# zju3dv/Mirror-NeRF

Measured on AMD Instinct MI355X. Metric: rendered rays/sec (primary+reflected), higher is better.
Workload: dtype f32 carried as hi/lo f16 pairs (f16 MFMA, f32 accumulate; max |diff| to the fp32 chain 3e-6)

## Files before the change

include/mnrf.h:

```cpp
#ifndef MNRF_H
#define MNRF_H

#include <stdint.h>

#ifdef __cplusplus
extern "C" {
#endif

#define MNRF_HOST

#define MNRF_OK 0
#define MNRF_ERR_ARG (-1)
#define MNRF_ERR_LAUNCH (-2)
#define MNRF_ERR_UNSUPPORTED (-3)

#define MNRF_N_PARAMS 32

#define MNRF_SIGMA_ONLY 1u
#define MNRF_GRAD_NORMAL 2u
#define MNRF_SPLIT_F16 4u

#define MNRF_TCNN_GRAD_F16 16u
#define MNRF_TCNN_GRAD_FIXED 512u
#define MNRF_TCNN_F16 256u
// ... 161 lines not shown
                     float bound, int64_t B, const float* xyz, int64_t xyz_stride, const float* rays, const float* z_vals,
                     int spr, float* planes, void* stream);

int mnrf_tcnn_encode_flags(const float* table, MNRF_HOST const int64_t* offsets17_host, double log2_per_level_scale, int base_resolution,
                           float bound, int64_t B, const float* xyz, int64_t xyz_stride, const float* rays, const float* z_vals,
                           int spr, float* planes, unsigned flags, void* stream);
int mnrf_tcnn_table_half(const float* table, int64_t entries, void* table_half, void* stream);

int mnrf_bench_gather(const void* table, int64_t table_bytes, int bytes_per_gather, int64_t n_threads, int iters, float* out,
                      void* stream);

#define MNRF_FUSED_WHITE_BACK 1u
#define MNRF_FUSED_RGB_DEPTH 2u
#define MNRF_FUSED_BLENDED_LEVEL 8u
int mnrf_fused_samples_per_ray(void);
int mnrf_field_composite_fused(float* packed, int64_t n_rays, const float* rays, const float* z_vals,
                               const float* dir_emb, int64_t dir_stride, int flags,
                               float* weights, float* opacity, float* rgb_map, float* depth, float* mirror_mask,
                               float* surf_normal, float* x_surface, void* stream);
int mnrf_field_composite_fused_pn(float* packed, int64_t n_rays, const float* rays, const float* z_vals,
                                  const float* dir_emb, int64_t dir_stride, int flags,
                                  float* weights, float* opacity, float* rgb_map, float* depth, float* mirror_mask,
                                  float* surf_normal, float* x_surface, float* pred_normal, void* stream);

int mnrf_split_convert_long(int on);
int mnrf_split2_probe(const float* x, int64_t n_pairs, int relu, int long_form, uint32_t* hi, uint32_t* lo, void* stream);

#define MNRF_TRAIN_PLANES 256u
#define MNRF_PLANES_Y_HALF 0x100000u
int64_t mnrf_train_planes_bytes(int64_t B);
int64_t mnrf_train_dy_planes_bytes(int64_t B);

int mnrf_field_backward_planes(float* packed, int64_t B, const float* xyz, int64_t xyz_stride,
                               const float* rays, const float* z_vals, int spr,
                               const float* g_sigma, const float* g_rgb, const float* g_pred_normal,
                               const float* g_is_mirror, const float* rgb, const float* pred_normal,
                               const float* is_mirror, const uint64_t* save_mask, const float* save_inv,
                               void* dy_planes, uint32_t* seedmax, float* d_xyz, float* d_dir, const float* keep_mirror,
                               unsigned flags ,
                               void* stream);

int64_t mnrf_dw_planes_workspace_floats(int n_eval, MNRF_HOST const int64_t* B);
int mnrf_dw_planes(int n_eval, const void* const* x_planes, const void* const* dy_planes, MNRF_HOST const int64_t* B,
                   const uint32_t* const* seedmax, float* workspace, float* const* d_params, int accumulate, void* stream);

int64_t mnrf_train_planes2_bytes(int64_t B);
// ... 310 lines not shown
```

mirror_nerf_amd/csrc/mnrf_render.hip:

```cpp
#include <hip/hip_runtime.h>
#include <stdint.h>
#include <stdio.h>
#include <string.h>

#include "../../include/mnrf.h"
#include "mnrf_error.h"
#include "mnrf_fill.h"
#include "mnrf_rays.h"

static thread_local char g_err[512] = "";

int mnrf_fail(int code, const char* msg) {
    snprintf(g_err, sizeof(g_err), "%s", msg);
    return code;
}

int mnrf_check_launch(const char* where) {
    hipError_t e = hipGetLastError();
    if (e != hipSuccess) {
        snprintf(g_err, sizeof(g_err), "%s: %s", where, hipGetErrorString(e));
        return MNRF_ERR_LAUNCH;
    }
    return MNRF_OK;
}

extern "C" const char* mnrf_last_error(void) { return g_err; }
extern "C" int mnrf_version(void) { return 1; }

namespace {

constexpr float EPS32 = 1.1920928955078125e-07f;

__device__ __forceinline__ long long live_rows(long long cap, const int* __restrict__ n_live) {
    if (!n_live) return cap;
    const long long v = *n_live;
    return v < 0 ? 0 : (v < cap ? v : cap);
}

__device__ __forceinline__ float wave_sum(float v) {
#pragma unroll
    for (int o = 32; o > 0; o >>= 1) v += __shfl_xor(v, o);
    return v;
}
#include "mnrf_composite.inc"

__global__ void embed_kernel(const float* __restrict__ x, long long n, int c, int n_freqs, float* __restrict__ out,
                             const int* __restrict__ n_live) {
    const long long i = (long long)blockIdx.x * blockDim.x + threadIdx.x;
    if (i >= live_rows(n, n_live) * c) return;
    const long long row = i / c;
    const int ch = (int)(i % c);
    const int ld = c * (2 * n_freqs + 1);
    const float v = x[i];
    float* o = out + row * ld;
    o[ch] = v;
    for (int f = 0; f < n_freqs; ++f) {
        float s, co;
        sincosf(ldexpf(v, f), &s, &co);
        o[c * (1 + 2 * f) + ch] = s;
        o[c * (2 + 2 * f) + ch] = co;
    }
}

__global__ void sample_coarse_kernel(const float* __restrict__ rays, long long n_rays, const float* __restrict__ z_steps,
                                     int ns, int use_disp, float perturb, const float* __restrict__ prand,
                                     float* __restrict__ z_out, const int* __restrict__ n_live) {
    const long long i = (long long)blockIdx.x * blockDim.x + threadIdx.x;
    if (i >= live_rows(n_rays, n_live) * ns) return;
    const long long r = i / ns;
    const int s = (int)(i % ns);
    const float near = rays[r * 8 + 6], far = rays[r * 8 + 7];
    auto zat = [&](int k) -> float {
        const float t = z_steps[k];
        if (!use_disp) return near * (1.f - t) + far * t;
        return 1.f / (1.f / near * (1.f - t) + 1.f / far * t);
    };
    float z = zat(s);
    if (perturb > 0.f) {
        const float lower = s == 0 ? z : 0.5f * (zat(s - 1) + z);
        const float upper = s == ns - 1 ? z : 0.5f * (z + zat(s + 1));
        z = lower + (upper - lower) * (perturb * prand[i]);
    }
    z_out[i] = z;
}

struct CompArgs {
    const float* rays; long long n_rays; int S;
    const float* sigma; const float* z; const float* noise; const float* rgb; const float* is_mirror;
    const float* pred_normal; const float* normal; int white_back;
    float* weights; float* opacity; float* rgb_map; float* depth; float* mirror_mask;
    float* surf_normal; float* surf_normal_grad; float* normal_dif; float* x_surface;
    const int* n_live;
};

struct CompGlobalSrc {
    const CompArgs& A;
    long long ray;
    __device__ __forceinline__ bool has_w() const { return false; }
    __device__ __forceinline__ float w(int) const { return 0.f; }
    __device__ __forceinline__ bool has_noise() const { return A.noise != nullptr; }
    __device__ __forceinline__ bool has_rgb() const { return A.rgb != nullptr; }
    __device__ __forceinline__ bool has_mirror() const { return A.is_mirror != nullptr; }
    __device__ __forceinline__ bool has_pn() const { return A.pred_normal != nullptr; }
    __device__ __forceinline__ bool has_gn() const { return A.normal != nullptr; }
    __device__ __forceinline__ float z(int s) const { return A.z[ray * A.S + s]; }
    __device__ __forceinline__ float sigma(int s) const { return A.sigma[ray * A.S + s]; }
// ... 242 lines not shown
    if (!live) ray = n_rays - 1;
    sample_fine_ray(z_coarse, weights, ray, live, S, u, u_per_ray, n_imp, z_fine);
}

__global__ __launch_bounds__(256) void composite_sample_kernel(CompArgs A, const float* __restrict__ u, int u_per_ray, int n_imp,
                                                               float* __restrict__ z_fine) {
    const int lane = threadIdx.x & 63;
    long long ray = (long long)blockIdx.x * 4 + (threadIdx.x >> 6);
    const long long n_rays = live_rows(A.n_rays, A.n_live);
    if ((long long)blockIdx.x * 4 >= n_rays) return;
    const bool live = ray < n_rays;
    if (live) {
        const CompGlobalSrc src{A, ray};
        const CompMaps out{A.weights + ray * A.S, A.opacity, A.rgb_map, A.depth, A.mirror_mask, A.surf_normal,
                           A.surf_normal_grad, A.normal_dif, A.x_surface, A.rays, A.white_back};
        composite_ray(src, A.S, lane, ray, out);
    }
    __threadfence_block();
    __syncthreads();
    if (!live) ray = n_rays - 1;
    sample_fine_ray(A.z, A.weights, ray, live, A.S, u, u_per_ray, n_imp, z_fine);
}

__global__ void threshold_kernel(float* __restrict__ m, long long n, int* __restrict__ any, const int* __restrict__ n_live) {
    const long long i = (long long)blockIdx.x * blockDim.x + threadIdx.x;
    bool nz = false;
    if (i < live_rows(n, n_live)) {
        float v = m[i];
        if (v > 0.5f) v = 1.f;
        else if (v < 0.5f) v = 0.f;
        m[i] = v;
        nz = v != 0.f;
    }
    if (__ballot(nz) != 0ull && (threadIdx.x & 63) == 0 && any) atomicOr(any, 1);
}

struct ReflArgs {
    const float* rays; const float* x_surface; const float* normal; const float* normal_noise; float noise_std;
    const float* mask; long long n; int compact; float near2;
    float* sec; int* index; int* count; float* reflect_dir;
    const int* n_live;
    int* slot;
};

__global__ __launch_bounds__(1024) void reflect_compact_kernel(ReflArgs A) {
    __shared__ int s_wave[16];
    __shared__ int s_base;
    const int tid = threadIdx.x, lane = tid & 63, wv = tid >> 6;
    if (tid == 0) s_base = 0;
    __syncthreads();
    A.n = live_rows(A.n, A.n_live);
    for (long long start = 0; start < A.n; start += 1024) {
        const long long i = start + tid;
// ... 24 lines not shown
        __syncthreads();
        int woff = 0, tot = 0;
        for (int k = 0; k < 16; ++k) { const int c = s_wave[k]; if (k < wv) woff += c; tot += c; }
        const int base = s_base;
        if (sel) {
            const long long p = base + woff + before;
            float* o = A.sec + p * 8;
            o[0] = A.x_surface[i * 3]; o[1] = A.x_surface[i * 3 + 1]; o[2] = A.x_surface[i * 3 + 2];
            o[3] = r[0]; o[4] = r[1]; o[5] = r[2];
            o[6] = A.near2;
            o[7] = A.rays[i * 8 + 7];
            A.index[p] = (int)i;
            if (A.slot) A.slot[i] = (int)p;
        } else if (in && A.slot) {
            A.slot[i] = -1;
        }
        __syncthreads();
        if (tid == 0) s_base = base + tot;
        __syncthreads();
    }
    if (tid == 0) *A.count = s_base;
}

__global__ __launch_bounds__(256) void reflect_all_kernel(ReflArgs A) {
    const long long i = (long long)blockIdx.x * blockDim.x + threadIdx.x;
    A.n = live_rows(A.n, A.n_live);
    if (i == 0) *A.count = (int)A.n;
    if (i >= A.n) return;
    float nv[3], wvv[3], r[3];
#pragma unroll
    for (int k = 0; k < 3; ++k) {
        nv[k] = A.normal[i * 3 + k];
        if (A.normal_noise) nv[k] = nv[k] + A.normal_noise[i * 3 + k] * A.noise_std;
        wvv[k] = -A.rays[i * 8 + 3 + k];
    }
    const float ninv = 1.f / sqrtf(fmaxf(nv[0] * nv[0] + nv[1] * nv[1] + nv[2] * nv[2], EPS32));
    const float winv = 1.f / sqrtf(fmaxf(wvv[0] * wvv[0] + wvv[1] * wvv[1] + wvv[2] * wvv[2], EPS32));
#pragma unroll
    for (int k = 0; k < 3; ++k) { nv[k] = nv[k] * ninv; wvv[k] = wvv[k] * winv; }
    const float c = wvv[0] * nv[0] + wvv[1] * nv[1] + wvv[2] * nv[2];
#pragma unroll
    for (int k = 0; k < 3; ++k) r[k] = 2.f * c * nv[k] - wvv[k];
    if (A.reflect_dir) { for (int k = 0; k < 3; ++k) A.reflect_dir[i * 3 + k] = r[k]; }
    float* o = A.sec + i * 8;
    o[0] = A.x_surface[i * 3]; o[1] = A.x_surface[i * 3 + 1]; o[2] = A.x_surface[i * 3 + 2];
    o[3] = r[0]; o[4] = r[1]; o[5] = r[2];
    o[6] = A.near2;
    o[7] = A.rays[i * 8 + 7];
    A.index[i] = (int)i;
    if (A.slot) A.slot[i] = (int)i;
}

__global__ void blend_all_kernel(const float* __restrict__ base, const float* __restrict__ sec, const float* __restrict__ mask,
                                 long long n, int c, int direct, float* __restrict__ out, float* __restrict__ refl,
                                 const int* __restrict__ n_live) {
    const long long i = (long long)blockIdx.x * blockDim.x + threadIdx.x;
    if (i >= live_rows(n, n_live) * c) return;
    const float m = mask[i / c];
    const float b = base[i];
    const float part = direct ? sec[i] : b;
    out[i] = m * part + (1.f - m) * b;
    if (refl) refl[i] = direct ? sec[i] : 0.f;
}

__global__ void blend_scatter_kernel(const float* __restrict__ base, const float* __restrict__ sec, const int* __restrict__ index,
                                     long long n_sec, const float* __restrict__ mask, int c, float* __restrict__ out,
                                     float* __restrict__ refl, const int* __restrict__ n_sec_live) {
    const long long j = (long long)blockIdx.x * blockDim.x + threadIdx.x;
    if (j >= live_rows(n_sec, n_sec_live) * c) return;
    const long long row = index[j / c];
    const int ch = (int)(j % c);
    const float m = mask[row];
    const float v = sec[j];
    out[row * c + ch] = m * v + (1.f - m) * base[row * c + ch];
    if (refl) refl[row * c + ch] = v;
}

__global__ void blend2_kernel(const float* __restrict__ base_a, const float* __restrict__ sec_a, const float* __restrict__ base_b,
                              const float* __restrict__ sec_b, const int* __restrict__ slot, const float* __restrict__ mask, long long n,
                              int c, float* __restrict__ out_a, float* __restrict__ out_b, const int* __restrict__ n_live) {
    const long long i = (long long)blockIdx.x * blockDim.x + threadIdx.x;
    if (i >= live_rows(n, n_live) * c) return;
    const long long row = i / c;
    const int ch = (int)(i % c);
    const float m = mask[row];
// ... 9 lines not shown
        out_b[i] = m * part + (1.f - m) * b;
    }
}
__global__ void blend2_backward_kernel(const float* __restrict__ g_out_a, const float* __restrict__ g_out_b, const int* __restrict__ slot,
                                       const float* __restrict__ mask, long long n, int c, float* __restrict__ g_base_a,
                                       float* __restrict__ g_sec_a, float* __restrict__ g_base_b, float* __restrict__ g_sec_b,
                                       const int* __restrict__ n_live) {
    const long long i = (long long)blockIdx.x * blockDim.x + threadIdx.x;
    if (i >= live_rows(n, n_live) * c) return;
    const long long row = i / c;
    const int ch = (int)(i % c);
    const float m = mask[row];
    const int sl = slot[row];
    if (g_out_a) {
        const float g = g_out_a[i];
        if (g_base_a) g_base_a[i] = (1.f - m) * g;
        if (g_sec_a && sl >= 0) g_sec_a[(long long)sl * c + ch] = m * g;
    }
    if (g_out_b) {
        const float g = g_out_b[i];
        if (g_base_b) g_base_b[i] = (1.f - m) * g;
        if (g_sec_b && sl >= 0) g_sec_b[(long long)sl * c + ch] = m * g;
    }
}

struct Pose { float m[12]; };

__global__ void generate_rays_kernel(int H, int W, float focal, Pose c2w, float near, float far, float* __restrict__ rays) {
    const long long p = (long long)blockIdx.x * blockDim.x + threadIdx.x;
    if (p >= (long long)H * W) return;
    mnrf_pinhole_ray((int)(p % W), (int)(p / W), H, W, focal, c2w.m, near, far, rays + p * 8);
}

__global__ void reflect_backward_kernel(const float* __restrict__ rays, const float* __restrict__ normal,
                                        const int* __restrict__ index, long long n_sec, const float* __restrict__ g_sec,
                                        float* __restrict__ g_xs, float* __restrict__ g_normal, float* __restrict__ g_rays,
                                        const int* __restrict__ n_sec_live) {
    const long long j = (long long)blockIdx.x * blockDim.x + threadIdx.x;
    if (j >= live_rows(n_sec, n_sec_live)) return;
    const long long i = index ? index[j] : j;
    float nv[3], wv[3], gr[3];
#pragma unroll
    for (int k = 0; k < 3; ++k) { nv[k] = normal[i * 3 + k]; wv[k] = -rays[i * 8 + 3 + k]; gr[k] = g_sec[j * 8 + 3 + k]; }
    const float nsq = nv[0] * nv[0] + nv[1] * nv[1] + nv[2] * nv[2];
    const float wsq = wv[0] * wv[0] + wv[1] * wv[1] + wv[2] * wv[2];
    const float ninv = 1.f / sqrtf(fmaxf(nsq, EPS32)), winv = 1.f / sqrtf(fmaxf(wsq, EPS32));
// ... 409 lines not shown
    if (n == 0) return MNRF_OK;
    if (!base || !mask || !out) return mnrf_fail(MNRF_ERR_ARG, "mnrf_blend_scatter: null pointer");
    if (n_sec > 0 && !sec) return mnrf_fail(MNRF_ERR_ARG, "mnrf_blend_scatter: sec is null");
    if (!index && n_sec != n) return mnrf_fail(MNRF_ERR_ARG, "mnrf_blend_scatter: without an index n_sec must equal n");
    hipStream_t s = (hipStream_t)stream;
    const int direct = index == nullptr;
    hipLaunchKernelGGL(blend_all_kernel, dim3(blocks_for(n * c, 256)), dim3(256), 0, s, base, sec, mask, (long long)n, c,
                       direct, out, reflect_out, n_live);
    if (!direct && n_sec > 0)
        hipLaunchKernelGGL(blend_scatter_kernel, dim3(blocks_for(n_sec * c, 256)), dim3(256), 0, s, base, sec, index,
                           (long long)n_sec, mask, c, out, reflect_out, n_sec_live);
    return mnrf_check_launch("mnrf_blend_scatter");
}
extern "C" int mnrf_blend_scatter(const float* base, const float* sec, const int32_t* index, int64_t n_sec,
                                  const float* mask, int64_t n, int c, float* out, float* reflect_out, void* stream) {
    return blend_scatter_impl(base, sec, index, n_sec, mask, n, c, out, reflect_out, nullptr, nullptr, stream);
}
extern "C" int mnrf_blend_scatter_n(const float* base, const float* sec, const int32_t* index, int64_t n_sec,
                                    const float* mask, int64_t n, int c, float* out, float* reflect_out,
                                    const int32_t* n_sec_live, const int32_t* n_live, void* stream) {
    return blend_scatter_impl(base, sec, index, n_sec, mask, n, c, out, reflect_out, n_sec_live, n_live, stream);
}

static int reflect_backward_impl(const float* rays, const float* normal, const int32_t* index, int64_t n_sec,
                                 const float* g_sec, int64_t n_rays, float* g_x_surface, float* g_normal, float* g_rays,
                                 const int32_t* n_sec_live, void* stream) {
    if (n_rays < 0 || n_sec < 0) return mnrf_fail(MNRF_ERR_ARG, "mnrf_reflect_backward: bad size");
    if (n_rays == 0) return MNRF_OK;
    if (!rays || !normal || !g_x_surface || !g_normal || !g_rays || (n_sec > 0 && !g_sec))
        return mnrf_fail(MNRF_ERR_ARG, "mnrf_reflect_backward: null pointer");
    hipStream_t s = (hipStream_t)stream;
    mnrf::zero_fill(s, g_x_surface, n_rays * 3 * sizeof(float), g_normal, n_rays * 3 * sizeof(float), g_rays, n_rays * 8 * sizeof(float));
    if (n_sec > 0)
        hipLaunchKernelGGL(reflect_backward_kernel, dim3(blocks_for(n_sec, 256)), dim3(256), 0, s, rays, normal, index, (long long)n_sec,
                           g_sec, g_x_surface, g_normal, g_rays, n_sec_live);
    return mnrf_check_launch("mnrf_reflect_backward");
}
extern "C" int mnrf_reflect_backward(const float* rays, const float* normal, const int32_t* index, int64_t n_sec,
                                     const float* g_sec, int64_t n_rays, float* g_x_surface, float* g_normal, float* g_rays,
                                     void* stream) {
    return reflect_backward_impl(rays, normal, index, n_sec, g_sec, n_rays, g_x_surface, g_normal, g_rays, nullptr, stream);
}
extern "C" int mnrf_reflect_backward_n(const float* rays, const float* normal, const int32_t* index, int64_t n_sec,
                                       const float* g_sec, int64_t n_rays, float* g_x_surface, float* g_normal, float* g_rays,
                                       const int32_t* n_sec_live, void* stream) {
    return reflect_backward_impl(rays, normal, index, n_sec, g_sec, n_rays, g_x_surface, g_normal, g_rays, n_sec_live, stream);
// ... 145 lines not shown
```

mirror_nerf_amd/recursion.py:

```python
import ctypes
import os
from collections import defaultdict
import weakref
from types import SimpleNamespace

import torch
from torch import nn

from . import _lib
from .mirror_nerf import Embedding, MirrorNeRF
from .dnerf import render_rays_dnerf
from .rendering import render_rays

RAY_FORWARD_OFFSET = 0.1
BLENDED_BREAK_EVEN = 0.37
_MIRROR_FRACTION = weakref.WeakKeyDictionary()
JITTER_RAYS = 262144

PLACE_MIRROR_PRESETS = {
    "plane_x": (
        ("livingroom", dict(position=0.0, normal=(-1.0, 0.0, 0.0), rect=(-1.0, 1.0, -0.5, 0.5))),
        ("washroom", dict(position=-1.0, normal=(1.0, 0.0, 0.0), rect=(-1.0, 1.0, -1.0, 0.75))),
        ("office", dict(position=1.0, normal=(1.0, 0.0, 0.0), rect=(-1.0, 1.0, -1.0, 0.75))),
        (None, dict(position=-1.0, normal=(1.0, 0.0, 0.0), rect=(-1.0, 1.0, -0.5, 0.5))),
# ... 637 lines not shown
    maps_only = bool(kwargs.get("maps_only", to_cpu == "maps"))
    rough = getattr(args, "app_control_mirror_roughness", False)
    batch_jitter = kwargs.get("batch_jitter", noise_iter is None)
    one_field = getattr(args, "only_one_field", False)
    fine_epoch = getattr(args, "only_one_field_fine_epoch", 2)
    sel = "fine" if (N_importance > 0 and not one_field) else "coarse"
    blend_mode = kwargs.get("blended_level", "auto")
    if blend_mode not in (True, False, "auto"):
        raise ValueError(f"blended_level must be True, False or 'auto', not {blend_mode!r}")
    mirror_fraction = _MIRROR_FRACTION.setdefault(models.get(sel, models["coarse"]), {})

    def draw(n, dev):
        if noise_iter is not None:
            return next(noise_iter).to(dev).float().contiguous()
        return torch.randn(n, 3, device=dev)

    def stage_a(rays_chunk, level, host_flags=None, slot=0):
        rgb_depth = 1 <= level == args.max_recursive_level and not rough
        can_blend = bool(level < args.max_recursive_level and trace_flag and test_time and blend_mode is not False
                         and not (rough or place or subst or objects or multi))
        evidence = mirror_fraction.get(level)
        blended = can_blend and (blend_mode is True or (evidence is not None and evidence >= BLENDED_BREAK_EVEN))
        count_it = can_blend and blend_mode is not True
        r = render_rays(models, embeddings, rays_chunk, N_samples, use_disp, 0, 0, N_importance, chunk,
                        white_back, test_time=test_time,
                        compute_normal=trace_flag and (not args.predict_normal),
                        only_one_field=one_field, only_one_field_fine_epoch=fine_epoch,
                        current_epoch=fine_epoch + 1, _guard=False, _maps_only=maps_only or rgb_depth,
                        _rgb_depth_only=rgb_depth, _blended_level=blended)
        r[f"rgb_{sel}_reflect"] = torch.zeros_like(r[f"rgb_{sel}"])
        r[f"depth_{sel}_reflect"] = torch.zeros_like(r[f"depth_{sel}"])
        if placed is not None and not object_chain:
            _merge_objects(r, rays_chunk, placed, args.near, used_k, placed_renderers)
        elif placed is not None:
            for k, o in enumerate(placed):
                _merge_object(r, rays_chunk, o["xform"], args.near, None if used_k is None else used_k[k:k + 1],
                              placed_renderers[k], o["bounds"])
        elif objects:
            _merge_object(r, rays_chunk, obj_xform, args.near, obj_used, render_object, obj_bounds)
        mask = None
        for key in (f"mirror_mask_{sel}", "mirror_mask_fine", "mirror_mask_coarse"):
            if key in r:
                mask = r[key]
                break
        last = level >= args.max_recursive_level or not (trace_flag or place or multi)
        edit = None
        if place and not last:
            edit = lambda flag: _place_mirror(r, rays_chunk, sel, plane, args.near, flag)
        if multi and level == 0:
            r["new_mirror_index"] = torch.full((rays_chunk.shape[0],), -1, dtype=torch.int32, device=rays_chunk.device)
        if multi and not last:
            edit = lambda flag: _place_mirrors(r, rays_chunk, sel, mirrors_packed, args.near, flag, r.get("new_mirror_index") if level == 0 else None)
        pending, any_mirror, counted = None, False, None
        if mask is not None:
            if host_flags is not None and not last and rays_chunk.shape[0]:
                pending = _threshold_async(mask, host_flags, slot, edit)
                if count_it:
                    host = host_counts[slot:slot + 1]
                    host.copy_(torch.count_nonzero(mask).view(1), non_blocking=True)
                    ev = torch.cuda.Event()
                    ev.record()
                    counted = (host, ev)
            else:
                any_mirror = _threshold_(mask, want_any=not last, edit=edit)
                if count_it and rays_chunk.shape[0]:
                    mirror_fraction[level] = (int(torch.count_nonzero(mask).item()) if any_mirror else 0) / rays_chunk.shape[0]
        return r, rays_chunk, level, mask, any_mirror, pending, counted

    def render_field(obj_rays, dnerf, time, field_models, field_embeddings):
        if dnerf is not None:
            d = obj_rays[:, 3:6]
            batch = torch.cat([obj_rays, torch.full_like(obj_rays[:, :1], time), d / torch.norm(d, dim=-1, keepdim=True)], -1)
            o = render_rays_dnerf(batch, **dict(dnerf, _frame_time=time))
            return {"rgb_fine": o["rgb_map"], "depth_fine": o["depth_map"], "opacity_fine": o["acc_map"]}
        return render_rays(field_models, field_embeddings, obj_rays, N_samples, use_disp, 0, 0, N_importance, chunk, white_back,
                           test_time=True, compute_normal=False, _guard=False, _maps_only=True, _rgb_depth_only=True)

    def render_object(obj_rays):
        return render_field(obj_rays, obj_dnerf, frame_time, obj_models, obj_embeddings)

    def placed_renderer(o):
        if o["kind"] == "d_nerf":
            return lambda obj_rays: render_field(obj_rays, o["field"], o["time"], None, None)
        field_models, field_embeddings = _object_system(o["field"])
        return lambda obj_rays: render_field(obj_rays, None, None, field_models, field_embeddings)

    placed_renderers = [placed_renderer(o) for o in placed] if placed is not None else None

    def recurse(rays_chunk, level):
        return stage_b(stage_a(rays_chunk, level))

    def stage_b(state):
        r, rays_chunk, level, mask, any_mirror, pending, counted = state
        if pending is not None:
            any_mirror = _flag_ready(pending)
        if counted is not None:
            counted[1].synchronize()
            mirror_fraction[level] = int(counted[0].item()) / rays_chunk.shape[0]
        N = rays_chunk.shape[0]
        dev = rays_chunk.device
        only_in = not (level < 1)
        trace = bool(mask is not None and any_mirror and (trace_flag or place or multi))
        if level >= args.max_recursive_level:
            trace = False
        if not trace or N == 0:
            return r
        mask = (mask != 0).float()
        normal = _pick_normal(r, sel)
        nn0 = draw(N, dev) if rough else None
        sec, index, rdir = _reflect(rays_chunk, r[f"x_surface_{sel}"], normal, mask, only_in, nn0, noise_std)
        r["reflect_direction"] = rdir
        if sec.shape[0] > 0:
            if subst:
                _transform_rays(sec, xform)
                r2 = render_rays(system_sub.models, system_sub.embeddings, sec.contiguous(), N_samples, use_disp, 0, 0,
                                 N_importance, chunk, white_back, test_time=test_time, compute_normal=False,
                                 only_one_field=one_field, only_one_field_fine_epoch=fine_epoch,
                                 current_epoch=fine_epoch + 1, _guard=False, _maps_only=True, _rgb_depth_only=True)
            else:
                r2 = recurse(sec.contiguous(), level + 1)
            if rough:
                times = args.trace_ray_times
                if batch_jitter and times > 0:
                    mj = max(1, r2[f"rgb_{sel}"].shape[0])
                    g = 0
                    while g < times:
                        n_g = max(1, min(times - g, JITTER_RAYS // mj))
# ... 14 lines not shown
                            if f"rgb_{typ}" in r2:
                                r2[f"rgb_{typ}"] = r2[f"rgb_{typ}"] + r3[f"rgb_{typ}"]
                for typ in ("coarse", "fine"):
                    if f"rgb_{typ}" in r2:
                        r2[f"rgb_{typ}"] = r2[f"rgb_{typ}"] / (times + 1)
            r[f"rgb_{sel}"], refl = _blend(r[f"rgb_{sel}"], r2[f"rgb_{sel}"], index, mask, True)
            r[f"rgb_{sel}_reflect"] = refl
            if only_in:
                d = torch.zeros_like(r[f"depth_{sel}"])
                d[index.long()] = r2[f"depth_{sel}"]
                r[f"depth_{sel}_reflect"] = d
            else:
                r[f"depth_{sel}_reflect"] = r2[f"depth_{sel}"]
        return r

    results = defaultdict(list)
    stage_maps = to_cpu == "maps" and rays.is_cuda
    staged, staged_rows, hold = {}, defaultdict(int), []
    copy_stream = _copy_stream(rays.device) if stage_maps else None
    starts = list(range(0, rays.shape[0], chunk))
    pipelined = rays.is_cuda and not rough and len(starts) > 1 and os.environ.get("MNRF_EVAL_PIPELINE", "1") != "0"
    host_flags = torch.zeros(2, dtype=torch.int32).pin_memory() if pipelined else None
    host_counts = torch.zeros(2, dtype=torch.int64).pin_memory() if pipelined else None
    ahead = stage_a(rays[:chunk].contiguous(), 0, host_flags, 0) if (pipelined and starts) else None
    for n_c, i in enumerate(starts):
        if pipelined:
            state = ahead
            ahead = stage_a(rays[starts[n_c + 1]:starts[n_c + 1] + chunk].contiguous(), 0, host_flags, (n_c + 1) % 2) \
                if n_c + 1 < len(starts) else None
            out = stage_b(state)
        else:
            out = recurse(rays[i:i + chunk].contiguous(), 0)
        if stage_maps:
            done = torch.cuda.Event()
            done.record()
            copy_stream.wait_event(done)
        for k, v in out.items():
            if to_cpu == "maps" or maps_only:
                if v.dim() <= 2 and (v.dim() == 1 or v.shape[1] <= 3):
                    if stage_maps:
                        buf = staged.get(k)
                        if buf is None:
                            buf = staged[k] = _pinned(k, rays.shape[0], tuple(v.shape[1:]), v.dtype)
                        r0 = staged_rows[k]
                        with torch.cuda.stream(copy_stream):
                            buf[r0:r0 + v.shape[0]].copy_(v, non_blocking=True)
# ... 29 lines not shown
```

mirror_nerf_amd/rendering.py:

```python
import torch

from . import _lib
from .autograd import CompositeFn, EmbedFn, FieldFn
from .mirror_nerf import field_forward
from .weights import params_of

__all__ = ["render_rays", "sample_pdf"]

_LINSPACE = {}


def _linspace01(n, device):
    key = (n, str(device))
    t = _LINSPACE.get(key)
    if t is None:
        t = torch.linspace(0, 1, n).to(device)
        _LINSPACE[key] = t
    return t


def _n_freqs(emb):
    n = getattr(emb, "N_freqs", None)
    if n is None:
        raise RuntimeError("embeddings must expose N_freqs (Embedding modules)")
# ... 50 lines not shown
        q.requires_grad for mdl in models.values() for q in params_of(mdl)))
    n_live = kwargs.get("_n_live")
    if n_live is not None and (not train or test_time):
        raise NotImplementedError("_n_live (device-side ray count) is a feature of the training path")

    comp_detach, cut_heads, keep_mirror = 0, 0, None
    if train:
        if kwargs.get("detach_density_for_mask_loss", False):
            comp_detach |= _lib.MNRF_DETACH_W_MASK
            cut_heads |= _lib.MNRF_CUT_MIRROR_HEAD
        elif kwargs.get("detach_density_outside_mirror_for_mask_loss", False) and kwargs.get("mirror_mask") is not None:
            mm = kwargs["mirror_mask"]
            gv = kwargs.get("_gt_valid")
            if (gv if gv is not None else not bool((mm < 0).any().item())):
                if mm.shape[0] != N or kwargs.get("_compacted"):
                    raise IndexError(f"detach_density_outside_mirror_for_mask_loss: mirror_mask has {mm.shape[0]} entries "
                                     f"for {N} rays (compacted reflected rays: use only_trace_rays_in_mirrors=False)")
                keep_mirror = mm.bool().float().contiguous()
        if kwargs.get("detach_density_for_normal_loss", False):
            comp_detach |= _lib.MNRF_DETACH_W_NORMAL
            cut_heads |= _lib.MNRF_CUT_NORMAL_HEAD

    fan = bool(train and not test_time and not hashgrid and N and N_samples >= 3 and "view_dir" not in kwargs and rays.shape[1] == 8)
    view = kwargs.get("view_dir", rays[:, 3:6])
    if fan:
        dir_emb = None
    elif hashgrid:
        dir_emb = view.float().contiguous()
    else:
        dir_emb = EmbedFn.apply(view, n_fd, n_live) if (train and view.requires_grad) else _embed(view.detach(), n_fd, n_live)

    z_steps = kwargs.get("_z_steps")
    z_steps = _linspace01(N_samples, dev) if z_steps is None else z_steps.float().contiguous()
    S_fine = N_samples + N_importance
    two_pass = train and N and N_importance > 0 and not kwargs.get("only_one_field", False) and kwargs.get("_z_fine") is None
    pool_u = pool_n = None
    share, box = kwargs.get("_rng_share") or (1, None)

    def pooled(kind, need, make):
        have = box.get(kind) if box is not None else None
        if have is None or have.numel() < need:
            have = make(need * (share if box is not None else 1))
        if box is not None:
            box[kind] = have[need:]
        return have[:need]
    if two_pass and perturb > 0 and kwargs.get("_perturb_rand") is None and kwargs.get("_u") is None:
        pool_u = pooled("u", N * (N_samples + N_importance), lambda k: torch.rand(k, device=dev))
    auto_noise = {}
    if two_pass and noise_std != 0 and kwargs.get("_noise_coarse") is None and kwargs.get("_noise_fine") is None:
        pool_n = pooled("n", N * (N_samples + S_fine), lambda k: torch.randn(k, device=dev))
        if noise_std != 1:
            pool_n = pool_n * noise_std
        auto_noise = {"_noise_coarse": pool_n[:N * N_samples].view(N, N_samples), "_noise_fine": pool_n[N * N_samples:].view(N, S_fine)}
    prand = None
    if perturb > 0:
        prand = kwargs.get("_perturb_rand")
        if prand is None:
            prand = pool_u[:N * N_samples].view(N, N_samples) if pool_u is not None else torch.rand(N, N_samples, device=dev)
        else:
            prand = prand.float().contiguous()
    per_pass = {}
    if fan:
        from .autograd import RayFanFn
        r_cf, r_ff, r_cc, r_fc, de_c, de_f, z_vals = RayFanFn.apply(rays, n_fd, z_steps, N_samples, bool(use_disp), float(perturb),
                                                                   prand, n_live)
        per_pass = {"_noise_coarse": (r_fc, r_cc, de_c), "_noise_fine": (r_ff, r_cf, de_f)}
    else:
        z_vals = f(N, N_samples)
        if N:
            _lib.check(L.mnrf_sample_coarse_n(p(rays), N, p(z_steps), N_samples, int(bool(use_disp)), float(perturb),
                                              p(prand), p(z_vals), p(n_live), _lib.stream()), "mnrf_sample_coarse")

    has_fine = "fine" in models
    results = {}

    def inference_fused(model, typ, z, blended=False):
        from . import mirror_nerf as _mn
        from .weights import folded_of
        if _mn.precision_of(model) != "split" or z.shape[1] != L.mnrf_fused_samples_per_ray():
            return False
        if blended:
            return inference_fused_blended(model, typ, z)
        rgb_depth = bool(kwargs.get("_rgb_depth_only"))
        has_m = not rgb_depth and getattr(model, "predict_mirror_mask", True)
        has_n = not rgb_depth and getattr(model, "predict_normal", True)
        opacity, rgb_map, depth = f(N), f(N, 3), f(N)
        xs = None if rgb_depth else f(N, 3)
        mask = f(N) if has_m else None
        sn = f(N, 3) if has_n else None
        flags = (_lib.MNRF_FUSED_WHITE_BACK if white_back else 0) | (_lib.MNRF_FUSED_RGB_DEPTH if rgb_depth else 0)
        if _mn.LAUNCH_LOG is not None:
            e0, e1 = torch.cuda.Event(enable_timing=True), torch.cuda.Event(enable_timing=True)
            e0.record()
        rc = L.mnrf_field_composite_fused(p(folded_of(model)), N, p(rays), p(z), p(dir_emb), dir_emb.shape[1], flags,
                                          None, p(opacity), p(rgb_map), p(depth), p(mask), p(sn), p(xs), _lib.stream())
        if rc == _lib.MNRF_ERR_UNSUPPORTED:
            return False
# ... 77 lines not shown
                if getattr(model, "predict_normal", True):
                    o["pred_normal"] = f(0, 3)
                if getattr(model, "predict_mirror_mask", True):
                    o["is_mirror"] = f(0)
                if compute_normal:
                    o["normal"] = f(0, 3)
        noise = kwargs.get(noise_key)
        if noise is not None:
            noise = (noise.float() * noise_std).contiguous()
        elif noise_std != 0:
            noise = torch.randn(N, S, device=dev)
            if noise_std != 1:
                noise = noise * noise_std
        weights, opacity = f(N, S), f(N)
        full = not sigma_only
        has_m, has_n = full and "is_mirror" in o, full and "pred_normal" in o
        rgb_map = f(N, 3) if full else None
        depth = f(N) if full else None
        mask = f(N) if has_m else None
        sn = f(N, 3) if has_n else None
        sng = f(N, 3) if (full and compute_normal) else None
        nd = f(N) if (has_n and compute_normal) else None
        xs = f(N, 3) if full else None
        if N:
            _lib.check(L.mnrf_composite(
                p(rays), N, S, p(o["sigma"]), p(z), p(noise), p(o.get("rgb")), p(o.get("is_mirror")),
                p(o.get("pred_normal")), p(o.get("normal")) if full else None, int(bool(white_back)),
                p(weights), p(opacity), p(rgb_map), p(depth), p(mask), p(sn), p(sng), p(nd), p(xs),
                _lib.stream()), "mnrf_composite")
        results[f"weights_{typ}"] = weights
        results[f"opacity_{typ}"] = opacity
        results[f"z_vals_{typ}"] = z
        if sigma_only:
            return
        results[f"rgb_{typ}"] = rgb_map
        results[f"depth_{typ}"] = depth
        if has_m:
            results[f"mirror_mask_{typ}"] = mask
        if compute_normal:
            results[f"normal_{typ}"] = o["normal"].view(N, S, 3)
            results[f"surface_normal_grad_{typ}"] = sng
        if has_n:
            results[f"pred_normal_{typ}"] = o["pred_normal"].view(N, S, 3)
            results[f"surface_normal_{typ}"] = sn
        if compute_normal and has_n:
            results[f"normal_dif_{typ}"] = nd
        results[f"_x_surface_{typ}"] = xs
# ... 105 lines not shown
```

Before: 1.914 million.

## Fuse per-level glue kernels into prologue, epilogue and blend launches for inference

Adds a level prologue kernel that computes coarse depths, the direction embedding and zeroes scratch words in one launch. It also adds an epilogue that thresholds the mirror mask, counts mirrors and builds reflected rays in one pass, and a simple blend kernel for the recursion level. At test time the Python recursion uses these in place of separate threshold, reflect, embed and zero-fill launches, and reads back mirror flags and counts through pinned memory. This cuts kernel launch and host overhead per chunk, at the cost of a more complex conditional path with many eligibility checks.

After: 1.919 million, median of 6. Within noise of the previous version (+0.3%).

```diff
diff --git a/include/mnrf.h b/include/mnrf.h
--- a/include/mnrf.h
+++ b/include/mnrf.h
@@ -207,6 +207,14 @@
                                   const float* dir_emb, int64_t dir_stride, int flags,
                                   float* weights, float* opacity, float* rgb_map, float* depth, float* mirror_mask,
                                   float* surf_normal, float* x_surface, float* pred_normal, void* stream);
+
+int mnrf_level_prologue(const float* rays, int64_t n_rays, const float* z_steps, int n_samples, int use_disp,
+                        int n_freqs_dir, float* z_vals, float* dir_emb, int32_t* zero_words, int n_zero_words, void* stream);
+int mnrf_level_epilogue(float* mask, int64_t n_rays, int32_t* flags, const float* rays, const float* x_surface,
+                        const float* normal, float near2, float* sec_rays, int32_t* index, int32_t* count,
+                        float* reflect_dir, void* stream);
+int mnrf_blend_level(const float* base, const float* sec, const float* mask, int64_t n, int c, float* out,
+                     float* reflect_out, void* stream);
 
 int mnrf_split_convert_long(int on);
 int mnrf_split2_probe(const float* x, int64_t n_pairs, int relu, int long_form, uint32_t* hi, uint32_t* lo, void* stream);
diff --git a/mirror_nerf_amd/csrc/mnrf_render.hip b/mirror_nerf_amd/csrc/mnrf_render.hip
--- a/mirror_nerf_amd/csrc/mnrf_render.hip
+++ b/mirror_nerf_amd/csrc/mnrf_render.hip
@@ -44,15 +44,7 @@
 }
 #include "mnrf_composite.inc"
 
-__global__ void embed_kernel(const float* __restrict__ x, long long n, int c, int n_freqs, float* __restrict__ out,
-                             const int* __restrict__ n_live) {
-    const long long i = (long long)blockIdx.x * blockDim.x + threadIdx.x;
-    if (i >= live_rows(n, n_live) * c) return;
-    const long long row = i / c;
-    const int ch = (int)(i % c);
-    const int ld = c * (2 * n_freqs + 1);
-    const float v = x[i];
-    float* o = out + row * ld;
+__device__ __forceinline__ void embed_channel(float v, int c, int ch, int n_freqs, float* __restrict__ o) {
     o[ch] = v;
     for (int f = 0; f < n_freqs; ++f) {
         float s, co;
@@ -62,11 +54,18 @@
     }
 }
 
-__global__ void sample_coarse_kernel(const float* __restrict__ rays, long long n_rays, const float* __restrict__ z_steps,
-                                     int ns, int use_disp, float perturb, const float* __restrict__ prand,
-                                     float* __restrict__ z_out, const int* __restrict__ n_live) {
-    const long long i = (long long)blockIdx.x * blockDim.x + threadIdx.x;
-    if (i >= live_rows(n_rays, n_live) * ns) return;
+__global__ void embed_kernel(const float* __restrict__ x, long long n, int c, int n_freqs, float* __restrict__ out,
+                             const int* __restrict__ n_live) {
+    const long long i = (long long)blockIdx.x * blockDim.x + threadIdx.x;
+    if (i >= live_rows(n, n_live) * c) return;
+    const long long row = i / c;
+    const int ch = (int)(i % c);
+    const int ld = c * (2 * n_freqs + 1);
+    embed_channel(x[i], c, ch, n_freqs, out + row * ld);
+}
+
+__device__ __forceinline__ float coarse_depth(const float* __restrict__ rays, const float* __restrict__ z_steps, long long i, int ns,
+                                              int use_disp, float perturb, const float* __restrict__ prand) {
     const long long r = i / ns;
     const int s = (int)(i % ns);
     const float near = rays[r * 8 + 6], far = rays[r * 8 + 7];
@@ -81,7 +80,15 @@
         const float upper = s == ns - 1 ? z : 0.5f * (z + zat(s + 1));
         z = lower + (upper - lower) * (perturb * prand[i]);
     }
-    z_out[i] = z;
+    return z;
+}
+
+__global__ void sample_coarse_kernel(const float* __restrict__ rays, long long n_rays, const float* __restrict__ z_steps,
+                                     int ns, int use_disp, float perturb, const float* __restrict__ prand,
+                                     float* __restrict__ z_out, const int* __restrict__ n_live) {
+    const long long i = (long long)blockIdx.x * blockDim.x + threadIdx.x;
+    if (i >= live_rows(n_rays, n_live) * ns) return;
+    z_out[i] = coarse_depth(rays, z_steps, i, ns, use_disp, perturb, prand);
 }
 
 struct CompArgs {
@@ -370,13 +377,17 @@
     sample_fine_ray(A.z, A.weights, ray, live, A.S, u, u_per_ray, n_imp, z_fine);
 }
 
+__device__ __forceinline__ float threshold_value(float v) {
+    if (v > 0.5f) v = 1.f;
+    else if (v < 0.5f) v = 0.f;
+    return v;
+}
+
 __global__ void threshold_kernel(float* __restrict__ m, long long n, int* __restrict__ any, const int* __restrict__ n_live) {
     const long long i = (long long)blockIdx.x * blockDim.x + threadIdx.x;
     bool nz = false;
     if (i < live_rows(n, n_live)) {
-        float v = m[i];
-        if (v > 0.5f) v = 1.f;
-        else if (v < 0.5f) v = 0.f;
+        const float v = threshold_value(m[i]);
         m[i] = v;
         nz = v != 0.f;
     }
@@ -447,11 +458,7 @@
     if (tid == 0) *A.count = s_base;
 }
 
-__global__ __launch_bounds__(256) void reflect_all_kernel(ReflArgs A) {
-    const long long i = (long long)blockIdx.x * blockDim.x + threadIdx.x;
-    A.n = live_rows(A.n, A.n_live);
-    if (i == 0) *A.count = (int)A.n;
-    if (i >= A.n) return;
+__device__ __forceinline__ void reflect_row(const ReflArgs& A, long long i) {
     float nv[3], wvv[3], r[3];
 #pragma unroll
     for (int k = 0; k < 3; ++k) {
@@ -472,20 +479,32 @@
     o[3] = r[0]; o[4] = r[1]; o[5] = r[2];
     o[6] = A.near2;
     o[7] = A.rays[i * 8 + 7];
-    A.index[i] = (int)i;
+    if (A.index) A.index[i] = (int)i;
     if (A.slot) A.slot[i] = (int)i;
 }
 
-__global__ void blend_all_kernel(const float* __restrict__ base, const float* __restrict__ sec, const float* __restrict__ mask,
-                                 long long n, int c, int direct, float* __restrict__ out, float* __restrict__ refl,
-                                 const int* __restrict__ n_live) {
-    const long long i = (long long)blockIdx.x * blockDim.x + threadIdx.x;
-    if (i >= live_rows(n, n_live) * c) return;
-    const float m = mask[i / c];
+__global__ __launch_bounds__(256) void reflect_all_kernel(ReflArgs A) {
+    const long long i = (long long)blockIdx.x * blockDim.x + threadIdx.x;
+    A.n = live_rows(A.n, A.n_live);
+    if (i == 0) *A.count = (int)A.n;
+    if (i >= A.n) return;
+    reflect_row(A, i);
+}
+
+__device__ __forceinline__ void blend_value(float m, const float* __restrict__ base, const float* __restrict__ sec, long long i,
+                                            int direct, float* __restrict__ out, float* __restrict__ refl) {
     const float b = base[i];
     const float part = direct ? sec[i] : b;
     out[i] = m * part + (1.f - m) * b;
     if (refl) refl[i] = direct ? sec[i] : 0.f;
+}
+
+__global__ void blend_all_kernel(const float* __restrict__ base, const float* __restrict__ sec, const float* __restrict__ mask,
+                                 long long n, int c, int direct, float* __restrict__ out, float* __restrict__ refl,
+                                 const int* __restrict__ n_live) {
+    const long long i = (long long)blockIdx.x * blockDim.x + threadIdx.x;
+    if (i >= live_rows(n, n_live) * c) return;
+    blend_value(mask[i / c], base, sec, i, direct, out, refl);
 }
 
 __global__ void blend_scatter_kernel(const float* __restrict__ base, const float* __restrict__ sec, const int* __restrict__ index,
@@ -541,6 +560,47 @@
         if (g_base_b) g_base_b[i] = (1.f - m) * g;
         if (g_sec_b && sl >= 0) g_sec_b[(long long)sl * c + ch] = m * g;
     }
+}
+
+
+struct PrologueArgs {
+    const float* rays; long long n_rays; const float* z_steps; int ns; int use_disp; int n_freqs;
+    float* z_out; float* dir_emb;
+    int* zero_words; int n_zero;
+};
+__global__ __launch_bounds__(256) void level_prologue_kernel(PrologueArgs A) {
+    const long long i = (long long)blockIdx.x * blockDim.x + threadIdx.x;
+    if (i < A.n_zero) A.zero_words[i] = 0;
+    if (i < A.n_rays * A.ns) A.z_out[i] = coarse_depth(A.rays, A.z_steps, i, A.ns, A.use_disp, 0.f, nullptr);
+    if (A.dir_emb && i < A.n_rays * 3) {
+        const long long row = i / 3;
+        const int ch = (int)(i % 3);
+        embed_channel(A.rays[row * 8 + 3 + ch], 3, ch, A.n_freqs, A.dir_emb + row * (3 * (2 * A.n_freqs + 1)));
+    }
+}
+
+__global__ __launch_bounds__(256) void level_epilogue_kernel(float* __restrict__ m, int* __restrict__ flags, ReflArgs A) {
+    const long long i = (long long)blockIdx.x * blockDim.x + threadIdx.x;
+    bool nz = false;
+    if (i < A.n) {
+        const float v = threshold_value(m[i]);
+        m[i] = v;
+        nz = v != 0.f;
+    }
+    const unsigned long long bal = __ballot(nz);
+    if (bal != 0ull && (threadIdx.x & 63) == 0) {
+        atomicOr(flags, 1);
+        atomicAdd(flags + 1, __popcll(bal));
+    }
+    if (i == 0) *A.count = (int)A.n;
+    if (i < A.n) reflect_row(A, i);
+}
+
+__global__ void blend_level_kernel(const float* __restrict__ base, const float* __restrict__ sec, const float* __restrict__ mask,
+                                   long long n, int c, float* __restrict__ out, float* __restrict__ refl) {
+    const long long i = (long long)blockIdx.x * blockDim.x + threadIdx.x;
+    if (i >= n * c) return;
+    blend_value(mask[i / c] != 0.f ? 1.f : 0.f, base, sec, i, 1, out, refl);
 }
 
 struct Pose { float m[12]; };
@@ -996,6 +1056,45 @@
     return blend_scatter_impl(base, sec, index, n_sec, mask, n, c, out, reflect_out, n_sec_live, n_live, stream);
 }
 
+extern "C" int mnrf_level_prologue(const float* rays, int64_t n_rays, const float* z_steps, int n_samples, int use_disp,
+                                   int n_freqs_dir, float* z_vals, float* dir_emb, int32_t* zero_words, int n_zero_words,
+                                   void* stream) {
+    if (n_rays < 0 || n_samples < 1 || n_freqs_dir < 0 || n_zero_words < 0) return mnrf_fail(MNRF_ERR_ARG, "mnrf_level_prologue: bad size");
+    if (n_rays == 0) return MNRF_OK;
+    if (!rays || !z_steps || !z_vals) return mnrf_fail(MNRF_ERR_ARG, "mnrf_level_prologue: null pointer");
+    if (n_zero_words > 0 && !zero_words) return mnrf_fail(MNRF_ERR_ARG, "mnrf_level_prologue: zero_words is null");
+    if (n_rays * (n_samples > 3 ? n_samples : 3) > 0x7fffffffLL * 256) return mnrf_fail(MNRF_ERR_ARG, "mnrf_level_prologue: too many rays for one launch");
+    PrologueArgs A{rays, (long long)n_rays, z_steps, n_samples, use_disp, n_freqs_dir, z_vals, dir_emb, zero_words, n_zero_words};
+    long long threads = n_rays * (n_samples > 3 ? n_samples : 3);
+    if (threads < n_zero_words) threads = n_zero_words;
+    hipLaunchKernelGGL(level_prologue_kernel, dim3(blocks_for(threads, 256)), dim3(256), 0, (hipStream_t)stream, A);
+    return mnrf_check_launch("mnrf_level_prologue");
+}
+
+extern "C" int mnrf_level_epilogue(float* mask, int64_t n_rays, int32_t* flags, const float* rays, const float* x_surface,
+                                   const float* normal, float near2, float* sec_rays, int32_t* index, int32_t* count,
+                                   float* reflect_dir, void* stream) {
+    if (n_rays < 0) return mnrf_fail(MNRF_ERR_ARG, "mnrf_level_epilogue: bad size");
+    if (n_rays == 0) return MNRF_OK;
+    if (!mask || !flags || !rays || !x_surface || !normal || !sec_rays || !count)
+        return mnrf_fail(MNRF_ERR_ARG, "mnrf_level_epilogue: null pointer");
+    if (n_rays > 0x7fffffffLL) return mnrf_fail(MNRF_ERR_ARG, "mnrf_level_epilogue: too many rays for one launch");
+    ReflArgs A{rays, x_surface, normal, nullptr, 0.f, nullptr, (long long)n_rays, 0, near2, sec_rays, index, count, reflect_dir,
+               nullptr, nullptr};
+    hipLaunchKernelGGL(level_epilogue_kernel, dim3(blocks_for(n_rays, 256)), dim3(256), 0, (hipStream_t)stream, mask, flags, A);
+    return mnrf_check_launch("mnrf_level_epilogue");
+}
+
+extern "C" int mnrf_blend_level(const float* base, const float* sec, const float* mask, int64_t n, int c, float* out,
+                                float* reflect_out, void* stream) {
+    if (n < 0 || c < 1) return mnrf_fail(MNRF_ERR_ARG, "mnrf_blend_level: bad size");
+    if (n == 0) return MNRF_OK;
+    if (!base || !sec || !mask || !out) return mnrf_fail(MNRF_ERR_ARG, "mnrf_blend_level: null pointer");
+    hipLaunchKernelGGL(blend_level_kernel, dim3(blocks_for(n * c, 256)), dim3(256), 0, (hipStream_t)stream, base, sec, mask,
+                       (long long)n, c, out, reflect_out);
+    return mnrf_check_launch("mnrf_blend_level");
+}
+
 static int reflect_backward_impl(const float* rays, const float* normal, const int32_t* index, int64_t n_sec,
                                  const float* g_sec, int64_t n_rays, float* g_x_surface, float* g_normal, float* g_rays,
                                  const int32_t* n_sec_live, void* stream) {
diff --git a/mirror_nerf_amd/recursion.py b/mirror_nerf_amd/recursion.py
--- a/mirror_nerf_amd/recursion.py
+++ b/mirror_nerf_amd/recursion.py
@@ -683,14 +683,23 @@
         evidence = mirror_fraction.get(level)
         blended = can_blend and (blend_mode is True or (evidence is not None and evidence >= BLENDED_BREAK_EVEN))
         count_it = can_blend and blend_mode is not True
+        glue = bool(level == 0 < args.max_recursive_level and trace_flag and test_time and glue_words is not None
+                    and rays_chunk.shape[0] and not (rough or place or subst or objects or multi))
+        words = glue_words[4 * slot:4 * slot + 4] if glue else None
         r = render_rays(models, embeddings, rays_chunk, N_samples, use_disp, 0, 0, N_importance, chunk,
                         white_back, test_time=test_time,
                         compute_normal=trace_flag and (not args.predict_normal),
                         only_one_field=one_field, only_one_field_fine_epoch=fine_epoch,
                         current_epoch=fine_epoch + 1, _guard=False, _maps_only=maps_only or rgb_depth,
-                        _rgb_depth_only=rgb_depth, _blended_level=blended)
-        r[f"rgb_{sel}_reflect"] = torch.zeros_like(r[f"rgb_{sel}"])
-        r[f"depth_{sel}_reflect"] = torch.zeros_like(r[f"depth_{sel}"])
+                        _rgb_depth_only=rgb_depth, _blended_level=blended, _level_scratch=words)
+        glue = bool(r.pop("_level_zeroed", False)) and glue and f"x_surface_{sel}" in r and f"mirror_mask_{sel}" in r \
+            and (f"surface_normal_{sel}" in r or f"surface_normal_grad_{sel}" in r)
+        if glue:
+            r[f"rgb_{sel}_reflect"] = torch.empty_like(r[f"rgb_{sel}"])
+            r[f"depth_{sel}_reflect"] = torch.empty_like(r[f"depth_{sel}"])
+        elif not rgb_depth:
+            r[f"rgb_{sel}_reflect"] = torch.zeros_like(r[f"rgb_{sel}"])
+            r[f"depth_{sel}_reflect"] = torch.zeros_like(r[f"depth_{sel}"])
         if placed is not None and not object_chain:
             _merge_objects(r, rays_chunk, placed, args.near, used_k, placed_renderers)
         elif placed is not None:
@@ -712,8 +721,22 @@
             r["new_mirror_index"] = torch.full((rays_chunk.shape[0],), -1, dtype=torch.int32, device=rays_chunk.device)
         if multi and not last:
             edit = lambda flag: _place_mirrors(r, rays_chunk, sel, mirrors_packed, args.near, flag, r.get("new_mirror_index") if level == 0 else None)
-        pending, any_mirror, counted = None, False, None
-        if mask is not None:
+        pending, any_mirror, counted, glued = None, False, None, None
+        if glue:
+            p, n, dev = _lib.ptr, rays_chunk.shape[0], rays_chunk.device
+            sec, rdir = _f(dev, n, 8), _f(dev, n, 3)
+            _lib.check(_lib.lib().mnrf_level_epilogue(
+                p(mask), n, p(words), p(rays_chunk), p(r[f"x_surface_{sel}"].contiguous()), p(_pick_normal(r, sel).contiguous()),
+                RAY_FORWARD_OFFSET, p(sec), None, p(words[2:3]), p(rdir), _lib.stream()), "mnrf_level_epilogue")
+            if host_flags is not None:
+                host = host_glue[2 * slot:2 * slot + 2]
+                host.copy_(words[:2], non_blocking=True)
+                ev = torch.cuda.Event()
+                ev.record()
+            else:
+                host, ev = words[:2].cpu(), None
+            glued = (sec, rdir, host, ev, count_it, words)
+        elif mask is not None:
             if host_flags is not None and not last and rays_chunk.shape[0]:
                 pending = _threshold_async(mask, host_flags, slot, edit)
                 if count_it:
@@ -726,7 +749,7 @@
                 any_mirror = _threshold_(mask, want_any=not last, edit=edit)
                 if count_it and rays_chunk.shape[0]:
                     mirror_fraction[level] = (int(torch.count_nonzero(mask).item()) if any_mirror else 0) / rays_chunk.shape[0]
-        return r, rays_chunk, level, mask, any_mirror, pending, counted
+        return r, rays_chunk, level, mask, any_mirror, pending, counted, glued
 
     def render_field(obj_rays, dnerf, time, field_models, field_embeddings):
         if dnerf is not None:
@@ -752,18 +775,40 @@
         return stage_b(stage_a(rays_chunk, level))
 
     def stage_b(state):
-        r, rays_chunk, level, mask, any_mirror, pending, counted = state
+        r, rays_chunk, level, mask, any_mirror, pending, counted, glued = state
         if pending is not None:
             any_mirror = _flag_ready(pending)
         if counted is not None:
             counted[1].synchronize()
             mirror_fraction[level] = int(counted[0].item()) / rays_chunk.shape[0]
+        if glued is not None:
+            if glued[3] is not None:
+                glued[3].synchronize()
+            any_mirror, n_mirror = (int(v) for v in glued[2].tolist())
+            any_mirror = bool(any_mirror)
+            if glued[4]:
+                mirror_fraction[level] = n_mirror / rays_chunk.shape[0]
         N = rays_chunk.shape[0]
         dev = rays_chunk.device
         only_in = not (level < 1)
         trace = bool(mask is not None and any_mirror and (trace_flag or place or multi))
         if level >= args.max_recursive_level:
             trace = False
+        if glued is not None:
+            if not trace:
+                r[f"rgb_{sel}_reflect"].zero_()
+                r[f"depth_{sel}_reflect"].zero_()
+                return r
+            sec, rdir = glued[0], glued[1]
+            r["reflect_direction"] = rdir
+            r2 = recurse(sec, level + 1)
+            base, part = r[f"rgb_{sel}"].contiguous(), r2[f"rgb_{sel}"].contiguous()
+            out = torch.empty_like(base)
+            _lib.check(_lib.lib().mnrf_blend_level(_lib.ptr(base), _lib.ptr(part), _lib.ptr(mask), N, 3, _lib.ptr(out),
+                                                   _lib.ptr(r[f"rgb_{sel}_reflect"]), _lib.stream()), "mnrf_blend_level")
+            r[f"rgb_{sel}"] = out
+            r[f"depth_{sel}_reflect"] = r2[f"depth_{sel}"]
+            return r
         if not trace or N == 0:
             return r
         mask = (mask != 0).float()
@@ -824,6 +869,8 @@
     pipelined = rays.is_cuda and not rough and len(starts) > 1 and os.environ.get("MNRF_EVAL_PIPELINE", "1") != "0"
     host_flags = torch.zeros(2, dtype=torch.int32).pin_memory() if pipelined else None
     host_counts = torch.zeros(2, dtype=torch.int64).pin_memory() if pipelined else None
+    glue_words = torch.empty(8, dtype=torch.int32, device=rays.device) if rays.is_cuda else None
+    host_glue = torch.zeros(4, dtype=torch.int32).pin_memory() if pipelined else None
     ahead = stage_a(rays[:chunk].contiguous(), 0, host_flags, 0) if (pipelined and starts) else None
     for n_c, i in enumerate(starts):
         if pipelined:
diff --git a/mirror_nerf_amd/rendering.py b/mirror_nerf_amd/rendering.py
--- a/mirror_nerf_amd/rendering.py
+++ b/mirror_nerf_amd/rendering.py
@@ -96,8 +96,9 @@
             cut_heads |= _lib.MNRF_CUT_NORMAL_HEAD
 
     fan = bool(train and not test_time and not hashgrid and N and N_samples >= 3 and "view_dir" not in kwargs and rays.shape[1] == 8)
+    glue = bool(not train and not hashgrid and N and perturb == 0 and "view_dir" not in kwargs and rays.shape[1] == 8)
     view = kwargs.get("view_dir", rays[:, 3:6])
-    if fan:
+    if fan or glue:
         dir_emb = None
     elif hashgrid:
         dir_emb = view.float().contiguous()
@@ -139,6 +140,11 @@
         r_cf, r_ff, r_cc, r_fc, de_c, de_f, z_vals = RayFanFn.apply(rays, n_fd, z_steps, N_samples, bool(use_disp), float(perturb),
                                                                    prand, n_live)
         per_pass = {"_noise_coarse": (r_fc, r_cc, de_c), "_noise_fine": (r_ff, r_cf, de_f)}
+    elif glue:
+        z_vals, dir_emb = f(N, N_samples), f(N, 3 * (2 * n_fd + 1))
+        scratch = kwargs.get("_level_scratch")
+        _lib.check(L.mnrf_level_prologue(p(rays), N, p(z_steps), N_samples, int(bool(use_disp)), n_fd, p(z_vals), p(dir_emb),
+                                         p(scratch), 0 if scratch is None else scratch.numel(), _lib.stream()), "mnrf_level_prologue")
     else:
         z_vals = f(N, N_samples)
         if N:
@@ -147,6 +153,9 @@
 
     has_fine = "fine" in models
     results = {}
+
+    if glue and kwargs.get("_level_scratch") is not None:
+        results["_level_zeroed"] = True
 
     def inference_fused(model, typ, z, blended=False):
         from . import mirror_nerf as _mn
@@ -270,7 +279,17 @@
         sng = f(N, 3) if (full and compute_normal) else None
         nd = f(N) if (has_n and compute_normal) else None
         xs = f(N, 3) if full else None
-        if N:
+        glue_u = resample_u() if (glue and noise is None and noise_key == "_noise_coarse") else None
+        if glue_u is not None:
+            glue_u = glue_u.float().contiguous()
+            zf = f(N, S + N_importance)
+            _lib.check(L.mnrf_composite_sample_n(
+                p(rays), N, S, p(o["sigma"]), p(z), None, p(o.get("rgb")), p(o.get("is_mirror")),
+                p(o.get("pred_normal")), p(o.get("normal")) if full else None, int(bool(white_back)),
+                p(weights), p(opacity), p(rgb_map), p(depth), p(mask), p(sn), p(sng), p(nd), p(xs),
+                p(glue_u), 1 if glue_u.dim() == 2 else 0, N_importance, p(zf), None, _lib.stream()), "mnrf_composite_sample_n")
+            results["_z_fine_fused"] = zf
+        elif N:
             _lib.check(L.mnrf_composite(
                 p(rays), N, S, p(o["sigma"]), p(z), p(noise), p(o.get("rgb")), p(o.get("is_mirror")),
                 p(o.get("pred_normal")), p(o.get("normal")) if full else None, int(bool(white_back)),
```
